# Lounes78/matcha-tts

Measured on AMD Instinct MI355X. Metric: mel-frames/sec + RTF, text->wav @10 ODE steps, LJSpeech model, 1/2/4/8 GPU, higher is better.
Workload: dtype bf16

## Files before the change

include/matcha_hip.h:

```cpp
#ifndef MATCHA_HIP_H
#define MATCHA_HIP_H

#include <stddef.h>
#include <stdint.h>

#ifdef __cplusplus
extern "C" {
#endif

#define MT_DTYPE_F32 0
#define MT_DTYPE_BF16 1
#define MT_SOLVER_EULER 0
#define MT_SOLVER_MIDPOINT 1

const char* mt_last_error(void);
int mt_abi_version(void);
int mt_build_experiments(void);
int mt_sched_count(void);
int mt_sched_get(int i, int* rec, int* wait, int* wait_first, int cap);

typedef struct mt_encoder mt_encoder;
int mt_encoder_create(int n_vocab, int n_channels, int filter_channels, int n_heads, int n_layers, int kernel_size,
                      int n_spks, int spk_emb_dim, int dp_filter_channels, int dp_kernel_size, int prenet, int dtype,
                      mt_encoder** out);
// ... 119 lines not shown
                      int rows, int C, float* dx, void* stream);
int mtt_snake_fwd(const float* x, const float* log_alpha, const float* log_beta, size_t n, int C, float* y,
                  void* stream);
int mtt_snake_bwd(const float* x, const float* log_alpha, const float* log_beta, const float* dy, size_t n, int C,
                  float* dx, float* galpha, float* gbeta, void* stream);
int mtt_softmax_fwd(const float* s, const float* kmask, const float* qmask, int BH, int H, int Tq, int Tk, float scale,
                    int mode, float* p, void* stream);
int mtt_softmax_bwd(const float* p, const float* dp, const float* kmask, const float* qmask, int BH, int H, int Tq,
                    int Tk, float scale, float* ds, void* stream);
int mtt_rope(float* x, int B, int T, int H, int dh, int d, const float* theta, int inverse, void* stream);
int mtt_embed_fwd(const int64_t* ids, size_t ntok, const float* table, int C, float scale, float* out, void* stream);
int mtt_embed_bwd(const int64_t* ids, size_t ntok, const float* dout, int V, int C, float scale, float* dtable,
                  void* stream);
int mtt_adam(float* p, const float* g, float* m, float* v, size_t n, const float* gscale, float lr, float beta1,
             float beta2, float eps, int step, void* stream);
int mtt_clip_factor(const float* sumsq, float max_norm, float inv_world, float* out, float* norm_out, void* stream);
int mtt_unscale(float* g, size_t n, float inv_scale, float* found, float* scratch, void* stream);

size_t mt_op_conv1d_workspace_bytes(int dtype, int cin, int cout, int k, int stride, int transposed);
int mt_op_conv1d(int dtype, const void* x, int B, int Tin, int cin, const float* W, const float* bias,
                 int cout, int k, int stride, int pad, int dil, int transposed, float slope, void* y,
                 int Tout, void* ws, size_t ws_bytes, void* stream);
int mt_op_conv1d_tile(int variant, int dtype, const void* x, int B, int Tin, int cin, const float* W,
                      const float* bias, int cout, int k, int stride, int pad, int dil, int transposed,
                      float slope, void* y, int Tout, void* ws, size_t ws_bytes, void* stream);
size_t mt_op_vconv_workspace_bytes(int cin, int cout, int k);
int mt_op_vconv(const void* x, int B, int L, int cin, const float* W, const float* bias, int cout, int k, int dil,
                int ef, const void* resid, void* y, void* y2, float slope, float div, const int32_t* lens, int pack,
                void* ws, size_t ws_bytes, void* stream);
int mt_vconv_set_rbconv(int enable);
int mt_vconv_set_ct(int enable);
int mt_vpair_set_kernels(int mask);
int mt_vocoder_set_post_fold(int enable);
int mt_vconv_set_actin(int enable);
int mt_ffn_set(int enable);
int mt_ffn_set_min_frames(int frames);
int mt_decoder_set_kernels(int mask);
int mt_op_attention(int dtype, const void* qkv, const float* mask, void* out, int B, int T, int heads,
                    void* stream);

#define MT_PROBE_RBFUSE_C64 1
#define MT_PROBE_RBFUSE_C32 2
#define MT_PROBE_VCONV 3
#define MT_PROBE_VCONV_DEC 4
int mt_probe_start(int site, int max_launches);
int mt_probe_pause(int paused);
int mt_probe_detail(int cap, double* ms, double* flops, double* bytes, int* tags);
int mt_probe_stop(int* launches, double* total_ms, double* flops, double* bytes, double peak_flops, double peak_bw,
                  double* roof_ms);

#define MT_VCONV_LOG_FIELDS 11
int mt_vconv_log_start(int capacity);
int mt_vconv_log_stop(int32_t* records, int capacity);
int mt_vconv_log_select(int families);

#ifdef __cplusplus
}
#endif
#endif
```

matcha-tts_amd/csrc/mt_capi.hip:

```cpp
#include <string.h>

#include <new>

#include "../../include/matcha_hip.h"
#include "mt_ffn.h"
#include "mt_model.h"
#include "mt_vconv.h"
#include "mt_vpair.h"
#include "mt_probe.h"
#include "mt_train.h"

namespace mt {
const char* last_error();
int denoise(const float* audio, int B, int L, const float* bias_spec, float strength, float* out, void* ws,
            size_t ws_bytes, hipStream_t st, const int* lens = nullptr, int lmul = 1);
size_t denoise_workspace_bytes(int B, int L);
int vconv_exp_flags();
int rbconv_exp_flags();
int ffn_exp_flags();
int vpair_exp_flags();
int stft_magnitude(const float* audio, int B, int L, float* mag, hipStream_t st);
int log_mel(const float* audio, int B, int L, const float* basis, float mean, float stdv, float* mel, hipStream_t st);
}

struct mt_encoder {
  mt::Encoder e;
};
struct mt_decoder {
  mt::Decoder d;
};
struct mt_vocoder {
  mt::Vocoder v;
};

using mt::set_error;

static int param_name(const mt::ParamList& L, int i, char* buf, int buflen) {
  MT_REQUIRE(i >= 0 && i < (int)L.names.size(), "param index %d out of range", i);
  MT_REQUIRE(buf && buflen > (int)L.names[i].size(), "param name buffer too small");
  memcpy(buf, L.names[i].c_str(), L.names[i].size() + 1);
  return 0;
}
static int param_shape(const mt::ParamList& L, int i, int64_t* shape, int maxdim) {
  MT_REQUIRE(i >= 0 && i < (int)L.names.size(), "param index %d out of range", i);
  const auto& s = L.shapes[i];
  MT_REQUIRE((int)s.size() <= maxdim, "shape buffer too small");
  for (size_t k = 0; k < s.size(); ++k) shape[k] = s[k];
  return (int)s.size();
}

extern "C" {

const char* mt_last_error(void) { return mt::last_error(); }
int mt_abi_version(void) { return 1; }
int mt_vpair_set_kernels(int mask) { return mt::vpair_set_kernels(mask); }
int mt_vocoder_set_post_fold(int enable) { return mt::vocoder_set_post_fold(enable); }
int mt_sched_count(void) { return mt::sched_count(); }
int mt_sched_get(int i, int* rec, int* wait, int* wait_first, int cap) {
  MT_REQUIRE(rec && wait && wait_first, "null buffer");
  const int S = mt::sched_get(i, rec, wait, wait_first, cap);
  MT_REQUIRE(S >= 0, "schedule %d: out of range or cap %d too small", i, cap);
  return S;
}
int mt_build_experiments(void) {
  return (mt::vconv_exp_flags() ? 1 : 0) | (mt::rbconv_exp_flags() ? 2 : 0) | (mt::ffn_exp_flags() ? 4 : 0) |
         (mt::vpair_exp_flags() ? 8 : 0);
}

int mt_encoder_create(int n_vocab, int n_channels, int filter_channels, int n_heads, int n_layers, int kernel_size,
                      int n_spks, int spk_emb_dim, int dp_filter_channels, int dp_kernel_size, int prenet, int dtype,
                      mt_encoder** out) {
  MT_REQUIRE(out, "null out");
  mt_encoder* h = new (std::nothrow) mt_encoder();
  MT_REQUIRE(h, "out of host memory");
  int rc = h->e.init(n_vocab, n_channels, filter_channels, n_heads, n_layers, kernel_size, n_spks, spk_emb_dim,
                     dp_filter_channels, dp_kernel_size, prenet, dtype);
  if (rc) {
    delete h;
    return rc;
  }
  *out = h;
  return 0;
}
void mt_encoder_destroy(mt_encoder* e) { delete e; }
int mt_encoder_num_params(const mt_encoder* e) { return e ? (int)e->e.params.names.size() : -1; }
int mt_encoder_param_name(const mt_encoder* e, int i, char* buf, int buflen) {
  MT_REQUIRE(e, "null encoder");
  return param_name(e->e.params, i, buf, buflen);
}
// ... 465 lines not shown
```

matcha-tts_amd/csrc/mt_probe.cpp:

```cpp
#include "mt_probe.h"
#include "mt_vconv.h"

#include <algorithm>
#include <mutex>
#include <vector>

namespace mt {
namespace {
std::mutex g_mu;
int g_site = PROBE_NONE;
std::vector<hipEvent_t> g_ev;
int g_n = 0, g_cap = 0;
double g_flops = 0, g_bytes = 0;
std::vector<double> g_lf, g_lb;
std::vector<int> g_lt;
bool g_open = false;
bool g_paused = false;

void release() {
  for (hipEvent_t e : g_ev) (void)hipEventDestroy(e);
  g_ev.clear();
  g_n = g_cap = 0;
  g_flops = g_bytes = 0;
  g_lf.clear();
  g_lb.clear();
  g_lt.clear();
  g_site = PROBE_NONE;
  g_open = false;
  g_paused = false;
}
}

bool probe_armed(int site) { return g_site != PROBE_NONE && g_site == site; }
bool probe_any_armed() { return g_site != PROBE_NONE; }

void probe_begin(int site, hipStream_t st) {
  if (!probe_armed(site)) return;
  std::lock_guard<std::mutex> lk(g_mu);
  if (g_n >= g_cap || g_open || g_paused) return;
  (void)hipEventRecord(g_ev[2 * g_n], st);
  g_open = true;
}

void probe_end(int site, hipStream_t st, double flops, double bytes, int tag) {
  if (!probe_armed(site)) return;
  std::lock_guard<std::mutex> lk(g_mu);
  if (!g_open) return;
  (void)hipEventRecord(g_ev[2 * g_n + 1], st);
  g_open = false;
  ++g_n;
  g_flops += flops;
  g_bytes += bytes;
  g_lf.push_back(flops);
  g_lb.push_back(bytes);
  g_lt.push_back(tag);
}

int probe_detail(int cap, double* ms, double* flops, double* bytes, int* tags) {
  std::lock_guard<std::mutex> lk(g_mu);
  const int n = std::min(cap, g_n);
  for (int i = 0; i < n; ++i) {
    float t = 0.f;
    if (hipEventSynchronize(g_ev[2 * i + 1]) != hipSuccess ||
        hipEventElapsedTime(&t, g_ev[2 * i], g_ev[2 * i + 1]) != hipSuccess) {
      set_error("probe: event timing failed");
      return -1;
    }
    if (ms) ms[i] = t;
    if (flops) flops[i] = g_lf[i];
    if (bytes) bytes[i] = g_lb[i];
    if (tags) tags[i] = g_lt[i];
  }
  return n;
}

int probe_start(int site, int max_launches) {
  std::lock_guard<std::mutex> lk(g_mu);
  release();
  MT_REQUIRE(site > PROBE_NONE && site <= PROBE_VCONV_DEC, "probe: unknown site %d", site);
  MT_REQUIRE(max_launches > 0 && max_launches <= (1 << 16), "probe: max_launches %d", max_launches);
  g_ev.resize(2 * (size_t)max_launches);
  for (hipEvent_t& e : g_ev) MT_CHECK_HIP(hipEventCreate(&e));
  g_cap = max_launches;
  g_site = site;
  return 0;
}

int probe_pause(bool paused) {
  std::lock_guard<std::mutex> lk(g_mu);
  g_paused = paused;
  return 0;
}

int probe_stop(int* launches, double* total_ms, double* flops, double* bytes, double peak_flops, double peak_bw,
               double* roof_ms) {
  std::lock_guard<std::mutex> lk(g_mu);
  double ms = 0, roof = 0;
  for (int i = 0; i < g_n; ++i)
    roof += 1e3 * std::max(peak_flops > 0 ? g_lf[i] / peak_flops : 0.0, peak_bw > 0 ? g_lb[i] / peak_bw : 0.0);
  int rc = 0;
  for (int i = 0; i < g_n && rc == 0; ++i) {
    float t = 0.f;
    if (hipEventSynchronize(g_ev[2 * i + 1]) != hipSuccess ||
        hipEventElapsedTime(&t, g_ev[2 * i], g_ev[2 * i + 1]) != hipSuccess) {
      set_error("probe: event timing failed");
      rc = -1;
    }
    ms += t;
  }
  if (launches) *launches = g_n;
  if (total_ms) *total_ms = ms;
  if (flops) *flops = g_flops;
  if (bytes) *bytes = g_bytes;
  if (roof_ms) *roof_ms = roof;
  release();
  return rc;
}

namespace {
std::vector<int> g_log;
int g_log_cap = 0;
bool g_log_on = false;
}

namespace {
struct SchedEntry {
  int rec[SCHED_FIELDS];
  SchedWaits waits;
};
std::vector<SchedEntry>& sched_table() {
  static std::vector<SchedEntry> t;
  return t;
}
}

int sched_register(const int (&rec)[SCHED_FIELDS], SchedWaits waits) {
  auto& t = sched_table();
  for (const auto& e : t)
    if (std::equal(e.rec, e.rec + SCHED_FIELDS, rec)) return 0;
  SchedEntry e;
  std::copy(rec, rec + SCHED_FIELDS, e.rec);
// ... 51 lines not shown
```

matcha-tts_amd/csrc/mt_probe.h:

```cpp
#pragma once
#include "mt_common.h"

namespace mt {

enum ProbeSite {
  PROBE_NONE = 0,
  PROBE_RBFUSE_C64 = 1,
  PROBE_RBFUSE_C32 = 2,
  PROBE_VCONV = 3,
  PROBE_VCONV_DEC = 4,
};

bool probe_armed(int site);
bool probe_any_armed();
void probe_begin(int site, hipStream_t st);
enum ProbeTag { PROBE_TAG_VCONV = 0, PROBE_TAG_VPAIR = 1, PROBE_TAG_VPAIR32 = 2, PROBE_TAG_RBFUSE = 3, PROBE_TAG_VPAIR128 = 4, PROBE_TAG_RBCONV = 5 };
void probe_end(int site, hipStream_t st, double flops, double bytes, int tag = PROBE_TAG_VCONV);
int probe_detail(int cap, double* ms, double* flops, double* bytes, int* tags);
int probe_start(int site, int max_launches);
int probe_pause(bool paused);
int probe_stop(int* launches, double* total_ms, double* flops, double* bytes, double peak_flops, double peak_bw,
               double* roof_ms);

constexpr int VCLOG_FIELDS = 11;
enum : int { VCLOG_CONV = 1, VCLOG_AUX = 2 };
void vclog_record(const int (&rec)[VCLOG_FIELDS], int family = VCLOG_CONV);
int vclog_select(int families);
int vclog_start(int cap);
int vclog_stop(int* out, int cap);
bool vclog_armed();

}
```

matcha-tts_amd/csrc/mt_vocoder.hip:

```cpp
#include <algorithm>
#include <type_traits>

#include "mt_model.h"
#include "mt_ragged.h"
#include "mt_rbfuse.h"
#include "mt_vconv.h"
#include "mt_vpair.h"

namespace mt {

constexpr int PC_N = 256;
__global__ __launch_bounds__(256) void post_conv_kernel(const bf16* __restrict__ x, int L,
                                                        const bf16* __restrict__ w, const float* __restrict__ bias,
                                                        float slope, float* __restrict__ out, const int* lens,
                                                        int lmul) {
  __shared__ __attribute__((aligned(16))) char rows[(PC_N + 16) * 64];
  const int b = blockIdx.y, f0 = blockIdx.x * PC_N, tid = threadIdx.x, lane = tid & 63, wave = tid >> 6;
  const bf16* xb = x + (size_t)b * L * 32;
  const int Lb = lens ? min(max(lens[b] * lmul, 0), L) : L;
  if (f0 >= Lb) {
    if (f0 + tid < L) out[(size_t)b * L + f0 + tid] = 0.f;
    return;
  }
  for (int e = tid; e < (PC_N + 6) * 4; e += 256) {
// ... 212 lines not shown
  for (int j = 0; j < nk; ++j)
    if (!rb_vp(i, j)) return false;
  return nk > 0;
}

bool Vocoder::stage_vp32(int i) const {
  const int nk = (int)rb_kernels.size();
  if (!pair || !fuse || vconv < 2 || !any_vc || dtype != BF16 || resblock != 1 || rb1[(size_t)i * nk].empty()) return false;
  for (int j = 0; j < nk; ++j)
    for (size_t q = 0; q < rb1[(size_t)i * nk + j].size(); ++q) {
      const GemmW& a = rb1[(size_t)i * nk + j][q];
      const GemmW& b = rb2[(size_t)i * nk + j][q];
      for (const GemmW* g : {&a, &b})
        if (g->cin != 32 || g->cout != 32 || g->Mpad != 32 || g->cin_pad != 32 || g->taps != g->k) return false;
      if (!vpair32_supported(a.k, a.dil) || b.k != a.k || b.dil != 1) return false;
    }
  return true;
}

static int g_postfold = -1;
int vocoder_post_fold() {
  if (g_postfold < 0) {
    const char* e = getenv("MT_POSTFOLD");
    g_postfold = e && e[0] == '0' ? 0 : 1;
  }
  return g_postfold;
}
int vocoder_set_post_fold(int enable) {
  const int prev = vocoder_post_fold();
  g_postfold = enable ? 1 : 0;
  return prev;
}

bool Vocoder::post_fold(int i) const {
  const int nk = (int)rb_kernels.size();
  return vocoder_post_fold() && dtype == BF16 && i + 1 == (int)ups.size() && stage_vp32(i) && post.cin == 32 &&
         post.k == 7 && post.cout == 1 && nk > 0 && (rb_kernels[nk - 1] - 1) / 2 <= 5;
}

int Vocoder::pair_resblock(const char* P, int i, int j, int B, int L, const char* X, char* XS, char* Tb, char* R,
                           char* RA, char* trash, bool act_out, hipStream_t st, const int* lens, float* wav) const {
  const int nk = (int)rb_kernels.size();
  const int C = rb1[(size_t)i * nk][0].cout;
  const bool c32 = C == 32;
  int rc;
  const std::vector<GemmW>& c1 = rb1[(size_t)i * nk + j];
  const std::vector<GemmW>& c2 = rb2[(size_t)i * nk + j];
  const int np = (int)c1.size();
  const char* state = X;
  for (int q = 0; q < np; ++q) {
    const bool last = q == np - 1;
    VPairArgs a{};
    a.x = (const bf16*)state;
    a.B = B;
    a.L = L;
    a.w1 = (const bf16*)(P + (c32 ? c1[q].w_off : c1[q].v_off));
    a.b1 = (const float*)(P + c1[q].b_off);
    a.w2 = (const bf16*)(P + (c32 ? c2[q].w_off : c2[q].v_off));
    a.b2 = (const float*)(P + c2[q].b_off);
    a.taps = c1[q].k;
    a.dil = c1[q].dil;
    a.div = (float)nk;
    a.slope = 0.1f;
    a.zero = (const bf16*)(P + zero_off);
    a.trash = (bf16*)trash;
    a.lens = lens;
    a.lmul = rate_upto(i + 1);
    int ef = 0;
    if (!last) {
      a.y = (bf16*)((q & 1) ? Tb : R);
    } else {
      a.y = (bf16*)XS;
      if (j > 0) ef |= VE_ACCUM;
      if (j == nk - 1) ef |= VE_DIV;
      if (j == nk - 1 && act_out) {
        a.y2 = (bf16*)RA;
        ef |= VE_DUAL | VE_Y2ONLY;
      }
      if (j == nk - 1 && wav && c32 && !act_out && j > 0) {
        a.post_w = (const bf16*)(P + post.w_off);
        a.post_b = (const float*)(P + post.b_off);
// ... 371 lines not shown
```

matcha-tts_amd/csrc/mt_vpair.h:

```cpp
#pragma once
#include "mt_ragged.h"
#include "mt_vconv.h"

namespace mt {

struct VPairArgs {
  const bf16* x;
  int B, L;
  const bf16* w1;
  const float* b1;
  const bf16* w2;
  const float* b2;
  int taps, dil;
  bf16* y;
  bf16* y2;
  float div, slope;
  const bf16* zero;
  bf16* trash;
  const int* lens;
  int lmul;
  const bf16* post_w;
  const float* post_b;
  float post_slope;
  float* wav;
// ... 60 lines not shown
  static constexpr int xwait_first = 2 * PW;
  static constexpr int accwait = 2 * (S - 1) + NXP;
};

template <int FAM, class SCH, int EF>
struct VpkReg {
  static int waits(int* w, int* wf, int cap) {
    if (cap < SCH::S + 1 || cap < 4) return -1;
    w[0] = -1;
    for (int s = 0; s < SCH::S; ++s) w[s + 1] = SCH::wait(s);
    wf[0] = SCH::wait_first0;
    wf[1] = SCH::xwait;
    wf[2] = SCH::xwait_first;
    wf[3] = SCH::accwait;
    return SCH::S;
  }
  static const int reg;
};
template <int FAM, class SCH, int EF>
const int VpkReg<FAM, SCH, EF>::reg =
    sched_register({FAM, SCH::NS, SCH::NXP, SCH::XSP, SCH::NACC, SCH::NST, SCH::NWS, EF, 0, 0, 0}, &VpkReg::waits);

enum : int { VPK_CTK = 1, VPK_CTK128 = 2, VPK_ALL = 3 };
int vpair_kernels();
int vpair_set_kernels(int mask);

bool vpair_supported(int C, int k, int d);
int launch_vpair(int ef, const VPairArgs& a, hipStream_t st);
bool vpair32_supported(int k, int d);
int launch_vpair32(int ef, const VPairArgs& a, hipStream_t st);
bool vpair128_supported(int k, int d);
int launch_vpair128(int ef, const VPairArgs& a, hipStream_t st);

}
```

matcha-tts_amd/matcha_hip/_lib.py:

```python
from __future__ import annotations

import ctypes
import os
from ctypes import POINTER, c_char_p, c_double, c_float, c_int, c_int64, c_size_t, c_uint, c_void_p

PKG_DIR = os.path.dirname(os.path.dirname(os.path.abspath(__file__)))
LIB_PATH = os.path.join(PKG_DIR, "libmatcha_hip.so")

DTYPE_F32 = 0
DTYPE_BF16 = 1
SOLVER_EULER = 0
SOLVER_MIDPOINT = 1

P = c_void_p

SIGNATURES = {
    "mt_last_error": (c_char_p, []),
    "mt_abi_version": (c_int, []),
    "mt_build_experiments": (c_int, []),
    "mt_sched_count": (c_int, []),
    "mt_sched_get": (c_int, [c_int, P, P, P, c_int]),
    "mt_encoder_create": (c_int, [c_int, c_int, c_int, c_int, c_int, c_int, c_int, c_int, c_int, c_int, c_int, c_int,
                                  POINTER(c_void_p)]),
    "mt_encoder_destroy": (None, [P]),
# ... 33 lines not shown
    "mt_vocoder_set_fusion": (c_int, [P, c_int]),
    "mt_vocoder_set_vconv": (c_int, [P, c_int]),
    "mt_vocoder_set_pair": (c_int, [P, c_int]),
    "mt_decoder_set_vconv": (c_int, [P, c_int]),
    "mt_vocoder_pack": (c_int, [P, POINTER(c_void_p), P, P]),
    "mt_vocoder_workspace_bytes": (c_size_t, [P, c_int, c_int]),
    "mt_vocoder_forward": (c_int, [P, P, P, c_int, c_int, P, P, c_size_t, P]),
    "mt_vocoder_forward_ragged": (c_int, [P, P, P, c_int, c_int, P, P, P, c_size_t, P]),
    "mt_vocoder_ragged_supported": (c_int, [P]),
    "mt_durations": (c_int, [P, P, c_float, c_int, c_int, P, P, P, P]),
    "mt_alignment": (c_int, [P, P, c_int, c_int, c_int, P, c_int, P, P, P, P]),
    "mt_denorm_crop": (c_int, [P, P, P, c_int, c_int, c_int, c_int, P, P]),
    "mt_denoise_workspace_bytes": (c_size_t, [c_int, c_int]),
    "mt_denoise": (c_int, [P, c_int, c_int, P, c_float, P, P, c_size_t, P]),
    "mt_denoise_ragged": (c_int, [P, c_int, c_int, P, c_int, P, c_float, P, P, c_size_t, P]),
    "mt_maximum_path_workspace_bytes": (c_size_t, [c_int, c_int, c_int]),
    "mt_decoder_step_times_workspace_bytes": (c_size_t, [P, c_int, c_int]),
    "mt_decoder_step_times": (c_int, [P, P, P, P, P, P, P, c_int, c_int, P, P, c_size_t, P]),
    "mt_maximum_path": (c_int, [P, P, P, c_int, c_int, c_int, P, P, c_size_t, P]),
    "mt_stft_magnitude": (c_int, [P, c_int, c_int, P, P]),
    "mt_log_mel": (c_int, [P, c_int, c_int, P, c_float, c_float, P, P]),
    "mt_op_conv1d_workspace_bytes": (c_size_t, [c_int, c_int, c_int, c_int, c_int, c_int]),
    "mt_op_conv1d": (c_int, [c_int, P, c_int, c_int, c_int, P, P, c_int, c_int, c_int, c_int, c_int,
                             c_int, c_float, P, c_int, P, c_size_t, P]),
    "mt_op_conv1d_tile": (c_int, [c_int, c_int, P, c_int, c_int, c_int, P, P, c_int, c_int, c_int, c_int, c_int,
                                  c_int, c_float, P, c_int, P, c_size_t, P]),
    "mt_op_vconv_workspace_bytes": (c_size_t, [c_int, c_int, c_int]),
    "mt_op_vconv": (c_int, [P, c_int, c_int, c_int, P, P, c_int, c_int, c_int, c_int, P, P, P, c_float, c_float,
                            P, c_int, P, c_size_t, P]),
    "mt_vconv_set_rbconv": (c_int, [c_int]),
    "mt_vconv_set_ct": (c_int, [c_int]),
    "mt_vpair_set_kernels": (c_int, [c_int]),
    "mt_vocoder_set_post_fold": (c_int, [c_int]),
    "mt_ffn_set": (c_int, [c_int]),
    "mt_vconv_set_actin": (c_int, [c_int]),
    "mt_ffn_set_min_frames": (c_int, [c_int]),
    "mt_decoder_set_kernels": (c_int, [c_int]),
    "mt_op_attention": (c_int, [c_int, P, P, P, c_int, c_int, c_int, P]),
    "mt_probe_start": (c_int, [c_int, c_int]),
    "mt_probe_pause": (c_int, [c_int]),
    "mt_probe_detail": (c_int, [c_int, P, P, P, P]),
    "mt_probe_stop": (c_int, [P, P, P, P, c_double, c_double, P]),
    "mtt_gemm": (c_int, [c_int, c_int, c_int, c_int, c_int, c_float, P, c_int, c_int64, P, c_int, c_int64, c_float,
                         P, c_int, c_int64, c_int, P, P, P, c_size_t, P]),
    "mtt_gemm_ex": (c_int, [c_int, c_int, c_int, c_int, c_int, c_int, c_float, P, c_int, c_int64, P, c_int, c_int64,
                            c_float, P, c_int, c_int64, c_int, P, P, P, c_size_t, P]),
    "mtt_gemm_workspace_bytes": (c_size_t, [c_int, c_int, c_int, c_int]),
    "mtt_im2col": (c_int, [P, P, c_int, c_int, c_int, c_int, c_int, c_int, c_int, c_int, P, P]),
    "mtt_col2im": (c_int, [P, P, c_int, c_int, c_int, c_int, c_int, c_int, c_int, c_int, P, c_int, P]),
    "mtt_ew": (c_int, [c_int, c_size_t, P, P, P, P, c_float, c_float, c_size_t, c_size_t, c_size_t, c_size_t,
                       c_size_t, c_size_t, c_int, P]),
    "mtt_copy_cols": (c_int, [P, c_int, c_int, P, c_int, c_int, c_int, c_int, c_int, P]),
    "mtt_seq_mask": (c_int, [P, c_int, c_int, P, P]),
    "mtt_colsum_scratch_floats": (c_size_t, [c_int, c_int, c_int]),
    "mtt_colsum": (c_int, [P, P, c_int, c_int, c_int, P, c_int, P, P]),
    "mtt_bcast_cols": (c_int, [P, c_int, P, c_int, c_int, c_int, c_int, P]),
    "mtt_segsum_cols_scratch_floats": (c_size_t, [c_int, c_int, c_int]),
    "mtt_segsum_cols": (c_int, [P, c_int, c_int, c_int, c_int, c_int, P, c_int, P, P]),
    "mtt_sum": (c_int, [P, P, c_size_t, P, P, P]),
    "mtt_dropout": (c_int, [P, c_size_t, c_float, c_uint, P, P]),
    "mtt_groupnorm_fwd": (c_int, [P, P, P, c_int, c_int, c_int, c_int, c_float, P, P, P, P]),
    "mtt_groupnorm_bwd": (c_int, [P, P, P, P, P, c_int, c_int, c_int, c_int, P, P, P, P]),
    "mtt_layernorm_fwd": (c_int, [P, P, P, c_int, c_int, c_float, P, P, P, P]),
    "mtt_layernorm_bwd": (c_int, [P, P, P, P, P, c_int, c_int, P, P]),
    "mtt_snake_fwd": (c_int, [P, P, P, c_size_t, c_int, P, P]),
    "mtt_snake_bwd": (c_int, [P, P, P, P, c_size_t, c_int, P, P, P, P]),
# ... 62 lines not shown
```

matcha-tts_amd/matcha_hip/runtime.py:

```python
from __future__ import annotations

import math
import time
from ctypes import byref, c_char_p, c_int, c_int64, c_void_p, create_string_buffer
from typing import Dict, List, Optional, Tuple

import torch

from ._lib import (DTYPE_BF16, DTYPE_F32, SOLVER_EULER, SOLVER_MIDPOINT, HipPathError, check, lib,
                   ptr, stream_handle)

_DTYPES = {"fp32": DTYPE_F32, "float32": DTYPE_F32, "f32": DTYPE_F32,
           "bf16": DTYPE_BF16, "bfloat16": DTYPE_BF16,
           "fp32x3": DTYPE_F32}


def dtype_code(precision: str) -> int:
    try:
        return _DTYPES[precision]
    except KeyError:
        raise ValueError(f"precision must be one of {sorted(set(_DTYPES))}, got {precision!r}")


def require_gpu(*tensors, what: str = "matcha_hip") -> None:
# ... 509 lines not shown
    if y is None:
        y = torch.empty((B, L, cout), dtype=torch.bfloat16, device=x.device)
    if (ef & 16) and y2 is None:
        y2 = torch.empty((B, L, cout), dtype=torch.bfloat16, device=x.device)
    if resid is not None:
        resid = resid.to(torch.bfloat16).contiguous()
    L_ = lib()
    nb = L_.mt_op_vconv_workspace_bytes(cin, cout, k)
    if ws is None or ws.numel() < nb:
        if not pack:
            raise ValueError("op_vconv: pack=False needs the workspace a packing call filled")
        ws = torch.empty(nb, dtype=torch.uint8, device=x.device)
    W, bias = f32c(W), f32c(bias)
    if lens is not None:
        lens = lens.to(device=x.device, dtype=torch.int32).contiguous()
    check(L_.mt_op_vconv(ptr(x), B, L, cin, ptr(W), ptr(bias), cout, k, dil, int(ef), ptr(resid), ptr(y), ptr(y2),
                         float(slope), float(div), ptr(lens), int(bool(pack)), ws.data_ptr(), ws.numel(),
                         stream_handle(x.device)), "op_vconv")
    return y, y2


def set_vconv_ct(enable: bool) -> bool:
    return bool(lib().mt_vconv_set_ct(int(bool(enable))))


def set_vpair_kernels(mask: int) -> int:
    return int(lib().mt_vpair_set_kernels(int(mask)))


def set_post_fold(enable) -> int:
    return int(lib().mt_vocoder_set_post_fold(int(bool(enable))))


def set_ffn(mode) -> int:
    return int(lib().mt_ffn_set(int(mode)))


def set_ffn_min_frames(frames: int) -> int:
    return int(lib().mt_ffn_set_min_frames(int(frames)))


def set_decoder_kernels(mask: int) -> int:
    return int(lib().mt_decoder_set_kernels(int(mask)))


def set_rbconv_actin(enable: bool) -> bool:
    return bool(lib().mt_vconv_set_actin(int(bool(enable))))


def set_rbconv(enable: bool) -> bool:
    return bool(lib().mt_vconv_set_rbconv(int(bool(enable))))


def op_attention(qkv: torch.Tensor, mask: torch.Tensor, heads: int, precision="fp32") -> torch.Tensor:
    require_gpu(qkv, mask, what="op_attention")
    dt = dtype_code(precision)
    et = torch.bfloat16 if dt == DTYPE_BF16 else torch.float32
    qkv = qkv.to(et).contiguous()
    B, T, _ = qkv.shape
    out = torch.empty((B, T, heads * 64), dtype=et, device=qkv.device)
    mask = f32c(mask.reshape(B, T))
    check(lib().mt_op_attention(dt, ptr(qkv), ptr(mask), ptr(out), B, T, heads, stream_handle(qkv.device)),
          "op_attention")
    return out


# ... 2 lines not shown

def probe_start(site: int, max_launches: int) -> None:
    check(lib().mt_probe_start(int(site), int(max_launches)), "probe_start")


def probe_pause(paused: bool) -> None:
    check(lib().mt_probe_pause(int(bool(paused))), "probe_pause")


PROBE_TAGS = ("vconv", "vpair", "vpair32", "rbfuse", "vpair128", "rbconv")


def probe_detail(cap: int = 4096) -> List[Dict[str, float]]:
    from ctypes import c_double
    ms, fl, by, tg = (c_double * cap)(), (c_double * cap)(), (c_double * cap)(), (c_int * cap)()
    n = lib().mt_probe_detail(int(cap), ms, fl, by, tg)
    if n < 0:
        check(n, "probe_detail")
    return [{"ms": ms[i], "flops": fl[i], "bytes": by[i], "kind": PROBE_TAGS[tg[i]]} for i in range(n)]


def probe_stop(peak_flops: float = 2.5e15, peak_bw: float = 8.0e12) -> Dict[str, float]:
    from ctypes import c_double
    n, ms, fl, by, roof = c_int(0), c_double(0), c_double(0), c_double(0), c_double(0)
    check(lib().mt_probe_stop(byref(n), byref(ms), byref(fl), byref(by), float(peak_flops), float(peak_bw),
                              byref(roof)), "probe_stop")
    return {"launches": n.value, "ms": ms.value, "flops": fl.value, "bytes": by.value, "roof_ms": roof.value}


VCONV_LOG_FIELDS = ("ef", "bm", "bn", "k1", "ntiles", "grid", "taps", "M", "cin", "B", "L")
PROJ_LOG = 0x20000
UNI_LOG_PART, UNI_LOG_VEC, UNI_LOG_APPLY = 0x40000, 0x80000, 0xC0000
FFN_LOG = 0x400000
LOG_CONV, LOG_AUX = 1, 2


def vconv_log_select(families: int) -> int:
    return int(lib().mt_vconv_log_select(int(families)))


def vconv_log_start(capacity: int = 65536) -> None:
    check(lib().mt_vconv_log_start(int(capacity)), "vconv_log_start")


def vconv_log_stop(capacity: int = 65536) -> List[Dict[str, int]]:
    buf = (c_int * (capacity * len(VCONV_LOG_FIELDS)))()
    n = lib().mt_vconv_log_stop(buf, int(capacity))
    k = len(VCONV_LOG_FIELDS)
    return [dict(zip(VCONV_LOG_FIELDS, buf[i * k:(i + 1) * k])) for i in range(n)]
```

Measured before the change: 827,900.

## Fuse three 32-channel vocoder resblock conv pairs into one chained kernel

```diff
diff --git a/include/matcha_hip.h b/include/matcha_hip.h
--- a/include/matcha_hip.h
+++ b/include/matcha_hip.h
@@ -175,6 +175,7 @@
 int mt_vconv_set_ct(int enable);
 int mt_vpair_set_kernels(int mask);
 int mt_vocoder_set_post_fold(int enable);
+int mt_vocoder_set_chain(int mode);
 int mt_vconv_set_actin(int enable);
 int mt_ffn_set(int enable);
 int mt_ffn_set_min_frames(int frames);
diff --git a/matcha-tts_amd/csrc/mt_capi.hip b/matcha-tts_amd/csrc/mt_capi.hip
--- a/matcha-tts_amd/csrc/mt_capi.hip
+++ b/matcha-tts_amd/csrc/mt_capi.hip
@@ -55,6 +55,7 @@
 int mt_abi_version(void) { return 1; }
 int mt_vpair_set_kernels(int mask) { return mt::vpair_set_kernels(mask); }
 int mt_vocoder_set_post_fold(int enable) { return mt::vocoder_set_post_fold(enable); }
+int mt_vocoder_set_chain(int mode) { return mt::vocoder_set_chain(mode); }
 int mt_sched_count(void) { return mt::sched_count(); }
 int mt_sched_get(int i, int* rec, int* wait, int* wait_first, int cap) {
   MT_REQUIRE(rec && wait && wait_first, "null buffer");
diff --git a/matcha-tts_amd/csrc/mt_probe.cpp b/matcha-tts_amd/csrc/mt_probe.cpp
--- a/matcha-tts_amd/csrc/mt_probe.cpp
+++ b/matcha-tts_amd/csrc/mt_probe.cpp
@@ -11,6 +11,8 @@
 int g_site = PROBE_NONE;
 std::vector<hipEvent_t> g_ev;
 int g_n = 0, g_cap = 0;
+int g_ne = 0;
+std::vector<int> g_le, g_ld;
 double g_flops = 0, g_bytes = 0;
 std::vector<double> g_lf, g_lb;
 std::vector<int> g_lt;
@@ -20,7 +22,9 @@
 void release() {
   for (hipEvent_t e : g_ev) (void)hipEventDestroy(e);
   g_ev.clear();
-  g_n = g_cap = 0;
+  g_n = g_cap = g_ne = 0;
+  g_le.clear();
+  g_ld.clear();
   g_flops = g_bytes = 0;
   g_lf.clear();
   g_lb.clear();
@@ -38,22 +42,28 @@
   if (!probe_armed(site)) return;
   std::lock_guard<std::mutex> lk(g_mu);
   if (g_n >= g_cap || g_open || g_paused) return;
-  (void)hipEventRecord(g_ev[2 * g_n], st);
+  (void)hipEventRecord(g_ev[2 * g_ne], st);
   g_open = true;
 }
 
-void probe_end(int site, hipStream_t st, double flops, double bytes, int tag) {
+void probe_end(int site, hipStream_t st, double flops, double bytes, int tag, int parts) {
   if (!probe_armed(site)) return;
   std::lock_guard<std::mutex> lk(g_mu);
   if (!g_open) return;
-  (void)hipEventRecord(g_ev[2 * g_n + 1], st);
+  (void)hipEventRecord(g_ev[2 * g_ne + 1], st);
   g_open = false;
-  ++g_n;
+  parts = std::max(1, std::min(parts, g_cap - g_n));
   g_flops += flops;
   g_bytes += bytes;
-  g_lf.push_back(flops);
-  g_lb.push_back(bytes);
-  g_lt.push_back(tag);
+  for (int i = 0; i < parts; ++i) {
+    g_lf.push_back(flops / parts);
+    g_lb.push_back(bytes / parts);
+    g_lt.push_back(tag);
+    g_le.push_back(g_ne);
+    g_ld.push_back(parts);
+  }
+  g_n += parts;
+  ++g_ne;
 }
 
 int probe_detail(int cap, double* ms, double* flops, double* bytes, int* tags) {
@@ -61,12 +71,13 @@
   const int n = std::min(cap, g_n);
   for (int i = 0; i < n; ++i) {
     float t = 0.f;
-    if (hipEventSynchronize(g_ev[2 * i + 1]) != hipSuccess ||
-        hipEventElapsedTime(&t, g_ev[2 * i], g_ev[2 * i + 1]) != hipSuccess) {
+    const int e = g_le[i];
+    if (hipEventSynchronize(g_ev[2 * e + 1]) != hipSuccess ||
+        hipEventElapsedTime(&t, g_ev[2 * e], g_ev[2 * e + 1]) != hipSuccess) {
       set_error("probe: event timing failed");
       return -1;
     }
-    if (ms) ms[i] = t;
+    if (ms) ms[i] = t / g_ld[i];
     if (flops) flops[i] = g_lf[i];
     if (bytes) bytes[i] = g_lb[i];
     if (tags) tags[i] = g_lt[i];
@@ -101,12 +112,13 @@
   int rc = 0;
   for (int i = 0; i < g_n && rc == 0; ++i) {
     float t = 0.f;
-    if (hipEventSynchronize(g_ev[2 * i + 1]) != hipSuccess ||
-        hipEventElapsedTime(&t, g_ev[2 * i], g_ev[2 * i + 1]) != hipSuccess) {
+    const int e = g_le[i];
+    if (hipEventSynchronize(g_ev[2 * e + 1]) != hipSuccess ||
+        hipEventElapsedTime(&t, g_ev[2 * e], g_ev[2 * e + 1]) != hipSuccess) {
       set_error("probe: event timing failed");
       rc = -1;
     }
-    ms += t;
+    ms += t / g_ld[i];
   }
   if (launches) *launches = g_n;
   if (total_ms) *total_ms = ms;
diff --git a/matcha-tts_amd/csrc/mt_probe.h b/matcha-tts_amd/csrc/mt_probe.h
--- a/matcha-tts_amd/csrc/mt_probe.h
+++ b/matcha-tts_amd/csrc/mt_probe.h
@@ -15,7 +15,7 @@
 bool probe_any_armed();
 void probe_begin(int site, hipStream_t st);
 enum ProbeTag { PROBE_TAG_VCONV = 0, PROBE_TAG_VPAIR = 1, PROBE_TAG_VPAIR32 = 2, PROBE_TAG_RBFUSE = 3, PROBE_TAG_VPAIR128 = 4, PROBE_TAG_RBCONV = 5 };
-void probe_end(int site, hipStream_t st, double flops, double bytes, int tag = PROBE_TAG_VCONV);
+void probe_end(int site, hipStream_t st, double flops, double bytes, int tag = PROBE_TAG_VCONV, int parts = 1);
 int probe_detail(int cap, double* ms, double* flops, double* bytes, int* tags);
 int probe_start(int site, int max_launches);
 int probe_pause(bool paused);
diff --git a/matcha-tts_amd/csrc/mt_vchain32.hip b/matcha-tts_amd/csrc/mt_vchain32.hip
--- /dev/null
+++ b/matcha-tts_amd/csrc/mt_vchain32.hip
@@ -0,0 +1,368 @@
+#include <algorithm>
+#include <type_traits>
+
+#include "mt_probe.h"
+#include "mt_vpair.h"
+
+namespace mt {
+
+namespace {
+constexpr int NT = 512, C = 32;
+constexpr int RB = C * 2;
+constexpr int MR = 16;
+constexpr int TAPW = C * RB;
+
+template <int K>
+struct Geom {
+  static_assert(K == 3 || K == 7, "kernel sizes whose six convs' weights fit beside the two row buffers");
+  static constexpr int FN = K == 3 ? 6 : 4;
+  static constexpr int WNC = 16 * FN;
+  static constexpr int ROWS = 8 * WNC;
+  static constexpr int BROWS = ROWS + 2 * MR;
+  static constexpr int NP = BROWS / 16;
+  static constexpr int BUF = BROWS * RB;
+  static constexpr int T_OFF = BUF, W_OFF = 2 * BUF, PAR_OFF = W_OFF + 6 * K * TAPW;
+  static constexpr int RAG_OFF = PAR_OFF + 6 * C * 4;
+  static constexpr int LDS_BYTES = RAG_OFF + RAG_LDS;
+  static_assert(LDS_BYTES <= 160 * 1024, "LDS budget");
+};
+
+__device__ __forceinline__ int swz(int r) { return (r >> 1) & 2; }
+
+__device__ __forceinline__ void glds16(const void* src, char* lds) {
+  __builtin_amdgcn_global_load_lds(src, (__attribute__((address_space(3))) void*)lds, 16, 0, 0);
+}
+
+__device__ __forceinline__ void wait_vmcnt(int n) {
+  if (n < 7) {
+    if (n < 2) asm volatile("s_waitcnt vmcnt(0)" ::: "memory");
+    else if (n < 4) asm volatile("s_waitcnt vmcnt(2)" ::: "memory");
+    else asm volatile("s_waitcnt vmcnt(4)" ::: "memory");
+  } else if (n < 15) {
+    if (n < 10) asm volatile("s_waitcnt vmcnt(7)" ::: "memory");
+    else asm volatile("s_waitcnt vmcnt(10)" ::: "memory");
+  } else {
+    if (n < 23) asm volatile("s_waitcnt vmcnt(15)" ::: "memory");
+    else if (n < 31) asm volatile("s_waitcnt vmcnt(23)" ::: "memory");
+    else asm volatile("s_waitcnt vmcnt(31)" ::: "memory");
+  }
+}
+
+__device__ __forceinline__ void barrier() {
+  __builtin_amdgcn_sched_barrier(0);
+  asm volatile("s_waitcnt lgkmcnt(0)" ::: "memory");
+  __builtin_amdgcn_s_barrier();
+  asm volatile("" ::: "memory");
+  __builtin_amdgcn_sched_barrier(0);
+}
+}
+
+template <int K, int EF>
+__global__ __launch_bounds__(NT) void vchain32_kernel(VChainArgs a) {
+  using GE = Geom<K>;
+  constexpr int FN = GE::FN, WNC = GE::WNC, ROWS = GE::ROWS, NP = GE::NP;
+  constexpr int T_OFF = GE::T_OFF, W_OFF = GE::W_OFF, PAR_OFF = GE::PAR_OFF, RAG_OFF = GE::RAG_OFF;
+  constexpr int HH = (K - 1) / 2;
+  __shared__ __attribute__((aligned(1024))) char smem[GE::LDS_BYTES];
+  const int tid = threadIdx.x, lane = tid & 63;
+  const int wave = __builtin_amdgcn_readfirstlane(tid >> 6);
+  const int g4 = lane >> 4, l16 = lane & 15, lrow = lane >> 2, lp = lane & 3;
+  const int L = a.L;
+  const int H = (a.dil[0] + a.dil[1] + a.dil[2] + 3) * HH;
+  const int BN = ROWS - 2 * H;
+  const int ntn = (L + BN - 1) / BN;
+  const bool rag = a.lens != nullptr;
+  int* rtc = reinterpret_cast<int*>(smem + RAG_OFF);
+  int* rlv = rtc + RAG_MAXB;
+  if (rag) {
+    rag_build(rtc, rlv, a.lens, a.lmul, L, 0, L, a.B, BN, tid);
+    __syncthreads();
+  }
+  const int ntiles = __builtin_amdgcn_readfirstlane(rag ? rtc[a.B - 1] : a.B * ntn);
+  const int G = gridDim.x, g = blockIdx.x;
+  const int gl = (G % 8 == 0) ? (g % 8) * (G / 8) + g / 8 : g;
+  const int nmine = gl < ntiles ? (ntiles - gl + G - 1) / G : 0;
+  if (nmine == 0) return;
+  for (int i = tid; i < 6 * C; i += NT) reinterpret_cast<float*>(smem + PAR_OFF)[i] = a.b[i / C][i % C];
+  if (tid < 2 * MR * 4) {
+    const int r = tid >> 2, row = r < MR ? r : ROWS + r;
+    *reinterpret_cast<u32x4*>(smem + T_OFF + row * RB + (tid & 3) * 16) = u32x4{0u, 0u, 0u, 0u};
+  }
+  __syncthreads();
+
+  int issued = 0, xmk = 0;
+  RagWalk walk;
+  auto tile_of = [&](int ti) __attribute__((always_inline)) {
+    const int tile = __builtin_amdgcn_readfirstlane(gl + ti * G);
+    if (rag) return walk.at(rtc, rlv, a.B, BN, tile);
+    RagTile t;
+    t.b = tile / ntn;
+    t.n0 = (tile - t.b * ntn) * BN;
+    t.lv = L;
+    return t;
+  };
+  RagTile nxt;
+  auto stage_weights = [&]() {
+    for (int j = wave; j < 12 * K; j += 8) {
+      const int cv = j / (2 * K), t = (j >> 1) - cv * K, r = (j & 1) * 16 + lrow;
+      glds16(a.w[cv] + ((size_t)r * K + t) * C + (lp ^ swz(r)) * 8, smem + W_OFF + (cv * K + t) * TAPW + (j & 1) * 1024);
+      ++issued;
+    }
+  };
+  const int xlane = lrow * RB + ((lp ^ swz(lrow)) * 16);
+  auto stage_x = [&](int ti) __attribute__((always_inline)) {
+    nxt = tile_of(ti);
+    const int b = __builtin_amdgcn_readfirstlane(nxt.b);
+    const int f0 = __builtin_amdgcn_readfirstlane(nxt.n0 - H - MR);
+    const unsigned nrec = (unsigned)__builtin_amdgcn_readfirstlane(nxt.lv) * RB;
+    const auto xr = __builtin_amdgcn_make_buffer_rsrc(const_cast<bf16*>(a.x + (size_t)b * L * C), (short)0, (int)nrec,
+                                                      0x00020000);
+#pragma unroll
+    for (int i = 0; i < (NP + 7) / 8; ++i) {
+      const int j = wave + 8 * i;
+      if (j < NP) {
+        __builtin_amdgcn_raw_ptr_buffer_load_lds(xr, (__attribute__((address_space(3))) void*)(smem + j * 1024), 16,
+                                                 (unsigned)(xlane + (f0 + 16 * j) * RB), 0, 0, 0);
+        ++issued;
+      }
+    }
+    xmk = issued;
+  };
+
+  auto swap16 = [](uint32_t& x, uint32_t& y) {
+    const auto r = __builtin_amdgcn_permlane16_swap(x, y, false, false);
+    x = r[0];
+    y = r[1];
+  };
+
+  f32x4 acc[2][FN];
+  struct Frag {
+    bf16x8 A[2], B[FN];
+  };
+  auto read_frag = [&](Frag& F, int cv, int t, const char* src, int rb0) __attribute__((always_inline)) {
+    const char* pa = smem + W_OFF + (cv * K + t) * TAPW + l16 * RB + ((g4 ^ swz(l16)) * 16);
+#pragma unroll
+    for (int f = 0; f < 2; ++f) F.A[f] = *reinterpret_cast<const bf16x8*>(pa + f * 16 * RB);
+#pragma unroll
+    for (int fn = 0; fn < FN; ++fn) {
+      const int rb = rb0 + fn * 16;
+      F.B[fn] = *reinterpret_cast<const bf16x8*>(src + rb * RB + ((g4 ^ swz(rb)) * 16));
+    }
+  };
+  auto mma_tap = [&](const Frag& F, auto first) __attribute__((always_inline)) {
+#pragma unroll
+    for (int fm = 0; fm < 2; ++fm)
+#pragma unroll
+      for (int fn = 0; fn < FN; ++fn)
+        acc[fm][fn] = mfma16(F.A[fm], F.B[fn], decltype(first)::value ? f32x4{0.f, 0.f, 0.f, 0.f} : acc[fm][fn]);
+    constexpr int NR = 2 + FN, NMF = 2 * FN;
+#pragma unroll
+    for (int i = 0; i < NR; ++i) {
+      __builtin_amdgcn_sched_group_barrier(0x008, 1, 0);
+      __builtin_amdgcn_sched_group_barrier(0x100, 1, 0);
+    }
+    __builtin_amdgcn_sched_group_barrier(0x008, NMF - NR, 0);
+  };
+  Frag F0, F1;
+  auto conv = [&](int cv, const char* src, int rb0, int tstride) __attribute__((always_inline)) {
+    read_frag(F0, cv, 0, src, rb0);
+    read_frag(F1, cv, 1, src, rb0 + tstride);
+    mma_tap(F0, std::true_type{});
+#pragma unroll
+    for (int t = 1; t < K; t += 2) {
+      read_frag(F0, cv, t + 1, src, rb0 + (t + 1) * tstride);
+      mma_tap(F1, std::false_type{});
+      if (t + 2 < K) read_frag(F1, cv, t + 2, src, rb0 + (t + 2) * tstride);
+      mma_tap(F0, std::false_type{});
+    }
+  };
+
+  stage_weights();
+  stage_x(0);
+
+  const float* par = reinterpret_cast<const float*>(smem + PAR_OFF);
+  const int ch16 = (g4 & 1) * 16 + (g4 >> 1) * 8;
+  const int qc = (g4 & 1) * 2 + (g4 >> 1);
+  for (int ti = 0; ti < nmine; ++ti) {
+    const int b = nxt.b, n0 = nxt.n0, Lt = nxt.lv;
+    const int fbase = n0 - H + wave * WNC + l16;
+    wait_vmcnt(issued - xmk);
+    barrier();
+    uint32_t res[FN][2][2];
+#pragma unroll
+    for (int fn = 0; fn < FN; ++fn) {
+      const int r = wave * WNC + fn * 16 + l16 + MR;
+      const u32x4 v = *reinterpret_cast<const u32x4*>(smem + r * RB + ((qc ^ swz(r)) * 16));
+      uint32_t rx0 = v[0], rx1 = v[1], ry0 = v[2], ry1 = v[3];
+      swap16(rx0, ry0);
+      swap16(rx1, ry1);
+      res[fn][0][0] = rx0, res[fn][0][1] = rx1, res[fn][1][0] = ry0, res[fn][1][1] = ry1;
+    }
+    barrier();
+    for (int e = tid; e < NP * 64; e += NT) {
+      u32x4 v = *reinterpret_cast<const u32x4*>(smem + e * 16);
+#pragma unroll
+      for (int w = 0; w < 4; ++w) v[w] = lrelu_pk(v[w], a.slope);
+      *reinterpret_cast<u32x4*>(smem + e * 16) = v;
+    }
+    barrier();
+    u32x4 yv[FN];
+    int ymk = 0;
+#pragma unroll
+    for (int q = 0; q < 3; ++q) {
+      const int d = a.dil[q];
+      if constexpr ((EF & VE_ACCUM) != 0) {
+        if (q == 2) {
+#pragma unroll
+          for (int fn = 0; fn < FN; ++fn) {
+            const int i = min(max(fbase + fn * 16, 0), L - 1);
+            asm volatile("global_load_dwordx4 %0, %1, off"
+                         : "=v"(yv[fn])
+                         : "v"(a.y + ((size_t)b * L + i) * C + ch16)
+                         : "memory");
+          }
+          issued += FN;
+          ymk = issued;
+        }
+      }
+      conv(2 * q, smem, wave * WNC + l16 + MR - d * HH, d);
+#pragma unroll
+      for (int fn = 0; fn < FN; ++fn) {
+        const int j = wave * WNC + fn * 16 + l16;
+        const int f = fbase + fn * 16;
+        const bool ok = f >= 0 && f < Lt;
+        uint32_t o[2][2];
+#pragma unroll
+        for (int h = 0; h < 2; ++h) {
+          const f32x4 b4 = *reinterpret_cast<const f32x4*>(par + 2 * q * C + h * 16 + 4 * g4);
+          o[h][0] = ok ? lrelu_pk_f(f32x2{acc[h][fn][0], acc[h][fn][1]} + f32x2{b4[0], b4[1]}, a.slope) : 0u;
+          o[h][1] = ok ? lrelu_pk_f(f32x2{acc[h][fn][2], acc[h][fn][3]} + f32x2{b4[2], b4[3]}, a.slope) : 0u;
+        }
+        swap16(o[0][0], o[1][0]);
+        swap16(o[0][1], o[1][1]);
+        *reinterpret_cast<u32x4*>(smem + T_OFF + (j + MR) * RB + ((qc ^ swz(j)) * 16)) =
+            u32x4{o[0][0], o[0][1], o[1][0], o[1][1]};
+      }
+      barrier();
+      if (q == 2 && ti + 1 < nmine) stage_x(ti + 1);
+      conv(2 * q + 1, smem + T_OFF, wave * WNC + l16 + MR - HH, 1);
+      if (q < 2) {
+#pragma unroll
+        for (int fn = 0; fn < FN; ++fn) {
+          const int j = wave * WNC + fn * 16 + l16;
+          const int f = fbase + fn * 16;
+          const bool ok = f >= 0 && f < Lt;
+          uint32_t o2[2][2];
+#pragma unroll
+          for (int h = 0; h < 2; ++h) {
+            const f32x4 b4 = *reinterpret_cast<const f32x4*>(par + (2 * q + 1) * C + h * 16 + 4 * g4);
+#pragma unroll
+            for (int u = 0; u < 2; ++u) {
+              f32x2 v = f32x2{acc[h][fn][2 * u], acc[h][fn][2 * u + 1]} + f32x2{b4[2 * u], b4[2 * u + 1]};
+              v = v + unpk_bf16(res[fn][h][u]);
+              const uint32_t o1 = ok ? pk_bf16(v) : 0u;
+              res[fn][h][u] = o1;
+              o2[h][u] = lrelu_pk(o1, a.slope);
+            }
+          }
+          swap16(o2[0][0], o2[1][0]);
+          swap16(o2[0][1], o2[1][1]);
+          *reinterpret_cast<u32x4*>(smem + (j + MR) * RB + ((qc ^ swz(j)) * 16)) =
+              u32x4{o2[0][0], o2[0][1], o2[1][0], o2[1][1]};
+        }
+        barrier();
+      }
+    }
+    if constexpr ((EF & VE_ACCUM) != 0) {
+      wait_vmcnt(issued - ymk);
+#pragma unroll
+      for (int fn = 0; fn < FN; ++fn) asm volatile("" : "+v"(yv[fn]));
+    }
+    const int bu = __builtin_amdgcn_readfirstlane(b);
+    const auto yr = __builtin_amdgcn_make_buffer_rsrc(a.y + (size_t)bu * L * C, (short)0, (int)((unsigned)L * RB), 0x00020000);
+#pragma unroll
+    for (int fn = 0; fn < FN; ++fn) {
+      const int j = wave * WNC + fn * 16 + l16;
+      uint32_t yx0 = 0, yx1 = 0, yy0 = 0, yy1 = 0;
+      if constexpr ((EF & VE_ACCUM) != 0) {
+        yx0 = yv[fn][0], yx1 = yv[fn][1], yy0 = yv[fn][2], yy1 = yv[fn][3];
+        swap16(yx0, yy0);
+        swap16(yx1, yy1);
+      }
+      uint32_t o1[2][2];
+#pragma unroll
+      for (int h = 0; h < 2; ++h) {
+        const f32x4 b4 = *reinterpret_cast<const f32x4*>(par + 5 * C + h * 16 + 4 * g4);
+        const uint32_t yy[2] = {h ? yy0 : yx0, h ? yy1 : yx1};
+#pragma unroll
+        for (int u = 0; u < 2; ++u) {
+          f32x2 v = f32x2{acc[h][fn][2 * u], acc[h][fn][2 * u + 1]} + f32x2{b4[2 * u], b4[2 * u + 1]};
+          v = v + unpk_bf16(res[fn][h][u]);
+          if constexpr ((EF & VE_ACCUM) != 0) v = unpk_bf16(yy[u]) + v;
+          o1[h][u] = pk_bf16(v);
+        }
+      }
+      swap16(o1[0][0], o1[1][0]);
+      swap16(o1[0][1], o1[1][1]);
+      const bool keep = j >= H && j < ROWS - H;
+      const unsigned vo = keep ? (unsigned)(((fbase + fn * 16) * C + ch16) * 2) : 0x80000000u;
+      __builtin_amdgcn_raw_buffer_store_b128(u32x4{o1[0][0], o1[0][1], o1[1][0], o1[1][1]}, yr, vo, 0, 0);
+    }
+    issued += FN;
+  }
+  asm volatile("s_waitcnt vmcnt(0)" ::: "memory");
+}
+
+bool vchain32_supported(int k, const int* dil) {
+  if (k != 3 && k != 7) return false;
+  for (int q = 0; q < 3; ++q)
+    if (dil[q] < 1 || dil[q] * (k - 1) / 2 > MR) return false;
+  const int H = (dil[0] + dil[1] + dil[2] + 3) * ((k - 1) / 2);
+  const int rows = k == 3 ? Geom<3>::ROWS : Geom<7>::ROWS;
+  return 4 * H <= rows;
+}
+
+static int cu_count() {
+  static int n = 0;
+  if (n == 0) {
+    int dev = 0;
+    if (hipGetDevice(&dev) != hipSuccess ||
+        hipDeviceGetAttribute(&n, hipDeviceAttributeMultiprocessorCount, dev) != hipSuccess || n <= 0)
+      n = 256;
+  }
+  return n;
+}
+
+int launch_vchain32(int ef, const VChainArgs& a, hipStream_t st) {
+  MT_REQUIRE(a.x && a.y && a.B > 0 && a.L > 0, "vchain32: null argument / empty");
+  for (int i = 0; i < 6; ++i) MT_REQUIRE(a.w[i] && a.b[i], "vchain32: conv %d weights / bias", i);
+  MT_REQUIRE(vchain32_supported(a.taps, a.dil), "vchain32: k %d d %d %d %d", a.taps, a.dil[0], a.dil[1], a.dil[2]);
+  MT_REQUIRE(a.y != a.x, "vchain32: y must not alias x (neighbour tiles read x's halo)");
+  MT_REQUIRE(!a.lens || a.B <= RAG_MAXB, "vchain32: ragged batch of %d > %d utterances", a.B, RAG_MAXB);
+  const int H = (a.dil[0] + a.dil[1] + a.dil[2] + 3) * ((a.taps - 1) / 2);
+  const int bn = (a.taps == 3 ? Geom<3>::ROWS : Geom<7>::ROWS) - 2 * H;
+  const long ntiles = (long)a.B * ((a.L + bn - 1) / bn);
+  const int G = (int)std::min<long>(ntiles, cu_count());
+  const double flops = 6.0 * 2.0 * C * C * a.taps * (double)a.B * a.L;
+  const double bytes = ((ef & VE_ACCUM) ? 3.0 : 2.0) * (2.0 * C * (double)a.B * a.L) + 6.0 * 2.0 * C * C * a.taps;
+  probe_begin(PROBE_VCONV, st);
+  if (a.taps == 3 && ef == 0) hipLaunchKernelGGL((vchain32_kernel<3, 0>), dim3(G), dim3(NT), 0, st, a);
+  else if (a.taps == 3 && ef == VE_ACCUM) hipLaunchKernelGGL((vchain32_kernel<3, VE_ACCUM>), dim3(G), dim3(NT), 0, st, a);
+  else if (a.taps == 7 && ef == 0) hipLaunchKernelGGL((vchain32_kernel<7, 0>), dim3(G), dim3(NT), 0, st, a);
+  else if (a.taps == 7 && ef == VE_ACCUM) hipLaunchKernelGGL((vchain32_kernel<7, VE_ACCUM>), dim3(G), dim3(NT), 0, st, a);
+  else {
+    set_error("vchain32: epilogue %d not compiled in", ef);
+    return -1;
+  }
+  MT_CHECK_HIP(hipGetLastError());
+  probe_end(PROBE_VCONV, st, flops, bytes, PROBE_TAG_VPAIR32, 3);
+  for (int q = 0; q < 3; ++q) {
+    const int rec[VCLOG_FIELDS] = {(q == 2 ? ef : 0) | 0x10000 | VCHAIN_LOG_BIT, C, bn, 0, (int)ntiles, G, a.taps, C, C, a.B, a.L};
+    vclog_record(rec);
+  }
+  const int rec[VCLOG_FIELDS] = {VCHAIN_LOG, C, bn, 0, (int)ntiles, G, a.taps, C, C, a.B, a.L};
+  vclog_record(rec, VCLOG_AUX);
+  return 0;
+}
+
+}
diff --git a/matcha-tts_amd/csrc/mt_vocoder.hip b/matcha-tts_amd/csrc/mt_vocoder.hip
--- a/matcha-tts_amd/csrc/mt_vocoder.hip
+++ b/matcha-tts_amd/csrc/mt_vocoder.hip
@@ -268,6 +268,20 @@
   return prev;
 }
 
+static int g_vchain = -1;
+int vocoder_chain() {
+  if (g_vchain < 0) {
+    const char* e = getenv("MT_VCHAIN");
+    g_vchain = e && e[0] >= '0' && e[0] <= '3' ? e[0] - '0' : 1;
+  }
+  return g_vchain;
+}
+int vocoder_set_chain(int mode) {
+  const int prev = vocoder_chain();
+  g_vchain = mode & 3;
+  return prev;
+}
+
 bool Vocoder::post_fold(int i) const {
   const int nk = (int)rb_kernels.size();
   return vocoder_post_fold() && dtype == BF16 && i + 1 == (int)ups.size() && stage_vp32(i) && post.cin == 32 &&
@@ -283,6 +297,29 @@
   const std::vector<GemmW>& c1 = rb1[(size_t)i * nk + j];
   const std::vector<GemmW>& c2 = rb2[(size_t)i * nk + j];
   const int np = (int)c1.size();
+  if (c32 && np == 3 && j < nk - 1 && c1[1].k == c1[0].k && c1[2].k == c1[0].k &&
+      (vocoder_chain() & (c1[0].k == 3 ? 1 : c1[0].k == 7 ? 2 : 0))) {
+    const int dil[3] = {c1[0].dil, c1[1].dil, c1[2].dil};
+    if (vchain32_supported(c1[0].k, dil)) {
+      VChainArgs a{};
+      a.x = (const bf16*)X;
+      a.B = B;
+      a.L = L;
+      for (int q = 0; q < 3; ++q) {
+        a.w[2 * q] = (const bf16*)(P + c1[q].w_off);
+        a.b[2 * q] = (const float*)(P + c1[q].b_off);
+        a.w[2 * q + 1] = (const bf16*)(P + c2[q].w_off);
+        a.b[2 * q + 1] = (const float*)(P + c2[q].b_off);
+        a.dil[q] = dil[q];
+      }
+      a.taps = c1[0].k;
+      a.y = (bf16*)XS;
+      a.slope = 0.1f;
+      a.lens = lens;
+      a.lmul = rate_upto(i + 1);
+      return launch_vchain32(j > 0 ? VE_ACCUM : 0, a, st);
+    }
+  }
   const char* state = X;
   for (int q = 0; q < np; ++q) {
     const bool last = q == np - 1;
diff --git a/matcha-tts_amd/csrc/mt_vpair.h b/matcha-tts_amd/csrc/mt_vpair.h
--- a/matcha-tts_amd/csrc/mt_vpair.h
+++ b/matcha-tts_amd/csrc/mt_vpair.h
@@ -116,4 +116,21 @@
 bool vpair128_supported(int k, int d);
 int launch_vpair128(int ef, const VPairArgs& a, hipStream_t st);
 
+struct VChainArgs {
+  const bf16* x;
+  int B, L;
+  const bf16* w[6];
+  const float* b[6];
+  int taps, dil[3];
+  bf16* y;
+  float slope;
+  const int* lens;
+  int lmul;
+};
+constexpr int VCHAIN_LOG_BIT = 0x800000, VCHAIN_LOG = 0x800000;
+bool vchain32_supported(int k, const int* dil);
+int launch_vchain32(int ef, const VChainArgs& a, hipStream_t st);
+int vocoder_chain();
+int vocoder_set_chain(int mode);
+
 }
diff --git a/matcha-tts_amd/matcha_hip/_lib.py b/matcha-tts_amd/matcha_hip/_lib.py
--- a/matcha-tts_amd/matcha_hip/_lib.py
+++ b/matcha-tts_amd/matcha_hip/_lib.py
@@ -89,6 +89,7 @@
     "mt_vconv_set_ct": (c_int, [c_int]),
     "mt_vpair_set_kernels": (c_int, [c_int]),
     "mt_vocoder_set_post_fold": (c_int, [c_int]),
+    "mt_vocoder_set_chain": (c_int, [c_int]),
     "mt_ffn_set": (c_int, [c_int]),
     "mt_vconv_set_actin": (c_int, [c_int]),
     "mt_ffn_set_min_frames": (c_int, [c_int]),
diff --git a/matcha-tts_amd/matcha_hip/runtime.py b/matcha-tts_amd/matcha_hip/runtime.py
--- a/matcha-tts_amd/matcha_hip/runtime.py
+++ b/matcha-tts_amd/matcha_hip/runtime.py
@@ -565,6 +565,10 @@
     return int(lib().mt_vocoder_set_post_fold(int(bool(enable))))
 
 
+def set_vchain(mode: int) -> int:
+    return int(lib().mt_vocoder_set_chain(int(mode)))
+
+
 def set_ffn(mode) -> int:
     return int(lib().mt_ffn_set(int(mode)))
 
@@ -633,6 +637,7 @@
 PROJ_LOG = 0x20000
 UNI_LOG_PART, UNI_LOG_VEC, UNI_LOG_APPLY = 0x40000, 0x80000, 0xC0000
 FFN_LOG = 0x400000
+VCHAIN_LOG_BIT = VCHAIN_LOG = 0x800000
 LOG_CONV, LOG_AUX = 1, 2
 
 
```

Measured after the change: 831,900, median of 6. About the same (+0.5%).
